# danieleschmidt/connectome-gnn-suite

Hardware: AMD Instinct MI355X
Metric: training graphs/sec, 3-layer GCN, batch=4096x360-ROI connectomes (higher is better)
Workload: dtype f32; 1 GPU; cfg4-headline-gcn-4096x360-h64; model=gcn, rois=360, ws_k=14, edges_per_graph=5040, hidden=64, layers=3, node_order=dataset, graphs_per_gpu=4096, global_batch=4096, optimizer=Adam lr1e-3 wd1e-4 (optim.Adam), impl=fused, launch=eager, bn=per-rank, rccl_ranks=0, parallelism=graph-sharded dp1

## Files before the change

### connectome_gnn_amd/csrc/fused_gcn.hip

```cpp
#include "common.h"
#include "agg_block.h"
#include "split_bf16.h"
#include "bn_tail.h"
#include "l0src.h"

#define PF_LD ld4
#define PF_ST st4
#define BW_LD ldnt4
#define BW_ST stnt4

#ifdef CGNN_STAMPS
__device__ unsigned long long g_stamps[1024 * 8 * 8];
#define CGNN_STAMP_DECL unsigned long long stamp_t_ = 0; (void)stamp_t_;
#define CGNN_STAMP_BEGIN() stamp_t_ = __builtin_amdgcn_s_memtime();
#define CGNN_STAMP(slot)                                                               \
  {                                                                                    \
    const unsigned long long now_ = __builtin_amdgcn_s_memtime();                      \
    if ((threadIdx.x & 63) == 0)                                                       \
      g_stamps[((size_t)blockIdx.x * 8 + (threadIdx.x >> 6)) * 8 + (slot)] += now_ - stamp_t_; \
    stamp_t_ = now_;                                                                   \
  }
#else
#define CGNN_STAMP_DECL
#define CGNN_STAMP_BEGIN()
// ... 340 lines not shown
  __shared__ __attribute__((aligned(16))) float bnab[2 * HID];
  __shared__ float disl[MAXR];
  const int lane = threadIdx.x & 63, wave = threadIdx.x >> 6, q = lane >> 4, j = lane & 15;
  const uint4* ent = static_cast<const uint4*>(t.ent_dst);
  constexpr int BPW = (MAXR / 16 + PF_NW - 1) / PF_NW;

  __shared__ __attribute__((aligned(16))) float b0l[FROM_P0 ? HID : 4];
  stage_split_weight<false>(wsp, W, PF_NTHR);
  for (int i = threadIdx.x; i < 2 * HID; i += PF_NTHR) bnab[i] = bn_prev[i];
  L0W w0;
  if (FROM_P0) {
    w0 = l0w_cols(l0, lane);
    for (int i = threadIdx.x; i < HID; i += PF_NTHR) b0l[i] = l0.b0[i];
  }
  const float4 bias4 = ld4(bias + 4 * j);
  double s1[4] = {0, 0, 0, 0}, s2[4] = {0, 0, 0, 0};

  constexpr int NPX = FROM_P0 ? 1 : 4;
  float4 px[BPW][NPX];
  float pd[BPW];
  auto request_block = [&](int tid, int u) {
    const int nb2 = t.tile_ptr[tid], nn2 = t.tile_ptr[tid + 1] - nb2;
    const int row = 16 * (wave + PF_NW * u) + j;
    pd[u] = 0.f;
#pragma unroll
    for (int c = 0; c < NPX; ++c) px[u][c] = make_float4(0.f, 0.f, 0.f, 0.f);
    if (row < nn2) {
      if (FROM_P0) {
        const float* src = l0.P0 + (int64_t)(nb2 + row) * L0_FP + q;
        px[u][0].x = src[0];
        px[u][0].y = src[4];
      } else {
        const float* src = Xin + (int64_t)(nb2 + row) * HID + 4 * q;
#pragma unroll
        for (int c = 0; c < NPX; ++c) px[u][c] = PF_LD(src + 16 * c);
      }
      pd[u] = t.dis[nb2 + row];
    }
  };
  auto request = [&](int tid) {
#pragma unroll
    for (int u = 0; u < BPW; ++u) request_block(tid, u);
  };
  if ((int)blockIdx.x < t.num_tiles) request(blockIdx.x);
  __syncthreads();

  for (int tid = blockIdx.x; tid < t.num_tiles; tid += gridDim.x) {
    const int base = t.tile_ptr[tid];
    const int n = t.tile_ptr[tid + 1] - base;
    const int nblk = (n + 15) >> 4;
    const int gb0 = t.tile_blk[tid];
    int boff[BPW], bwid[BPW];
#pragma unroll
    for (int k = 0; k < BPW; ++k) {
      boff[k] = bwid[k] = 0;
      const int bb = cgnn_uniform(wave) + PF_NW * k;
      if (bb < nblk) {
        boff[k] = t.blk_off_dst[gb0 + bb];
        bwid[k] = (t.blk_off_dst[gb0 + bb + 1] - boff[k]) >> 4;
      }
    }
    MetaRegs pre;
    if (wave < nblk) pre = meta_issue<true>(ent + (boff[0] >> 1), bwid[0], q, j);

    const int nxt = tid + gridDim.x;
#pragma unroll
    for (int u = 0; u < BPW; ++u) {
      const int b = wave + PF_NW * u;
      if (b >= nblk) break;
      const int row = 16 * b + j;
      const bool live = row < n;
      f32x4 acc[4] = {{0, 0, 0, 0}, {0, 0, 0, 0}, {0, 0, 0, 0}, {0, 0, 0, 0}};
#pragma unroll
      for (int ms = 0; ms < 2; ++ms) {
        float4 xc[2];
#pragma unroll
        for (int h2 = 0; h2 < 2; ++h2) {
          const int c = 2 * ms + h2;
          uint32_t keep = 0xFu;
          if (use_drop) {
            keep = drop_bits(drop, (uint32_t)(base + row), (uint32_t)(4 * c + q));
            if (mask_out && live) mask_out[(int64_t)(base + row) * 16 + 4 * c + q] = (uint8_t)keep;
          }
          float4 f;
          float4 yraw = px[u][c < NPX ? c : 0];
          if (FROM_P0) {
            const float4 bq = ld4(b0l + 16 * c + 4 * q);
            const l0_f32x4 y0 = l0_mfma(w0.a[c], w0.b[c], px[u][0].x, px[u][0].y, l0_f32x4{bq.x, bq.y, bq.z, bq.w});
            yraw = make_float4(y0[0], y0[1], y0[2], y0[3]);
          }
          xc[h2] = scale4(act4(yraw, ld4(bnab + 16 * c + 4 * q), ld4(bnab + HID + 16 * c + 4 * q),
                               keep, drop.scale, f), pd[u]);
        }
        const Split8 a = split8(xc[0], xc[1]);
#pragma unroll
        for (int tj = 0; tj < 4; ++tj) {
          const uint4 bh = wsp[((0 * 2 + ms) * 4 + tj) * 64 + lane];
          const uint4 bm = wsp[((1 * 2 + ms) * 4 + tj) * 64 + lane];
          const uint4 bl = wsp[((2 * 2 + ms) * 4 + tj) * 64 + lane];
          acc[tj] = mfma_split(a, bh, bm, bl, acc[tj]);
        }
        __builtin_amdgcn_sched_barrier(0);
      }
#pragma unroll
      for (int r = 0; r < 4; ++r)
        st4(tile + (16 * b + 4 * q + r) * HID + 4 * j, make_float4(acc[0][r], acc[1][r], acc[2][r], acc[3][r]));
      if (q == 0) disl[row] = pd[u];
      if (nxt < t.num_tiles) request_block(nxt, u);
    }
    if (nxt < t.num_tiles) {
#pragma unroll
      for (int u = 0; u < BPW; ++u)
        if (wave + PF_NW * u >= nblk) request_block(nxt, u);
    }
    __syncthreads();

#pragma unroll
    for (int u = 0; u < BPW; ++u) {
      const int b = wave + PF_NW * u;
      if (b >= nblk) break;
      float4 ag[4];
      agg_block<CGNN_PF_G, true>(tile, pre, ent + (boff[u] >> 1), bwid[u], q, j, ag);
      if (u + 1 < BPW && b + PF_NW < nblk) pre = meta_issue<true>(ent + (boff[u + 1 < BPW ? u + 1 : u] >> 1), bwid[u + 1 < BPW ? u + 1 : u], q, j);
#pragma unroll
      for (int it = 0; it < 4; ++it) {
        const int row = 16 * b + 4 * q + it;
        if (row < n) {
          const float4 a = scale4(ag[it], disl[row]);
          const float4 y = make_float4(a.x + bias4.x, a.y + bias4.y, a.z + bias4.z, a.w + bias4.w);
          PF_ST(Y + (int64_t)(base + row) * HID + 4 * j, y);
          s1[0] += y.x; s1[1] += y.y; s1[2] += y.z; s1[3] += y.w;
          s2[0] += (double)y.x * y.x; s2[1] += (double)y.y * y.y;
          s2[2] += (double)y.z * y.z; s2[3] += (double)y.w * y.w;
        }
      }
    }
    __syncthreads();
  }
  if (tail.acc) {
    double* red = reinterpret_cast<double*>(tile);
    reduce_stats<double, PF_NW>(s1, s2, red, red + PF_NW * 128);
    bn_tail_run(tail, red + PF_NW * 128, reinterpret_cast<int*>(red + PF_NW * 128 + 128), [](int) { return 0.f; });
  } else if (stat_slab) {
    reduce_stats<double, PF_NW>(s1, s2, reinterpret_cast<double*>(tile), stat_slab + (int64_t)blockIdx.x * 128);
  }
}

struct PoolIn {
  const float* dP;
  const int32_t* node_graph;
  const int32_t* gptr;
  const uint8_t* mask_cur;
};


template <int MAXR, bool FIRST, bool POOLIN, bool XP0 = false, int NW = NWAVE>
__global__ void __launch_bounds__(NW * 64) k_gcn_bwd(
    cgnn_tiles t, PoolIn pin, cgnn_l0src l0, const float* __restrict__ dZ, const float* __restrict__ Y,
    const float* __restrict__ bn, const float* __restrict__ bwc,
    const float* __restrict__ Xprev , int F0,
    const float* __restrict__ bn_prev, DropCfg drop, int use_drop,
    const uint8_t* __restrict__ mask_prev, const float* __restrict__ W,
    float* __restrict__ dZprev, double* __restrict__ s_slab, float* __restrict__ dW_slab,
    double* __restrict__ db_slab, cgnn_bn_tail tail) {
  __shared__ __attribute__((aligned(16))) float tile[MAXR * HID];
  __shared__ __attribute__((aligned(16))) float stg_all[NW * STG_FLOATS];
  __shared__ uint4 wsp[FIRST ? 1 : WSP_FRAGS];
  __shared__ float disl[MAXR];
  const int lane = threadIdx.x & 63, wave = threadIdx.x >> 6, q = lane >> 4, j = lane & 15;
  float* stg = stg_all + wave * STG_FLOATS;
  const uint4* ent = static_cast<const uint4*>(t.ent_src);

  if (!FIRST) stage_split_weight<true>(wsp, W, (NW * 64));
  __shared__ __attribute__((aligned(16))) float bnl[FIRST ? 4 : 4 * HID];
  if (!FIRST) {
    for (int i = threadIdx.x; i < 4 * HID; i += (NW * 64)) bnl[i] = bn_prev[i];
  }
  L0W w0;
  float4 b0q = make_float4(0.f, 0.f, 0.f, 0.f);
  if (XP0) {
    w0 = l0w_quad(l0, threadIdx.x & 63);
    b0q = ld4(l0.b0 + 4 * (threadIdx.x & 15));
  }
  f32x4 dw[4][FIRST ? 1 : 4];
#pragma unroll
  for (int a = 0; a < 4; ++a)
#pragma unroll
    for (int b2 = 0; b2 < (FIRST ? 1 : 4); ++b2) dw[a][b2] = f32x4{0, 0, 0, 0};
  float db[4] = {0, 0, 0, 0};
  float s1[4] = {0, 0, 0, 0}, s2[4] = {0, 0, 0, 0};
  CGNN_STAMP_DECL

  for (int tid = blockIdx.x; tid < t.num_tiles; tid += gridDim.x) {
    CGNN_STAMP_BEGIN()
    const int base = t.tile_ptr[tid];
    const int n = t.tile_ptr[tid + 1] - base;
    const int nblk = (n + 15) >> 4;
    const int gb0 = t.tile_blk[tid];
    const int uw = cgnn_uniform(wave);
    int off0 = 0, width = 0;
    if (uw < nblk) {
      off0 = t.blk_off_src[gb0 + uw];
      width = (t.blk_off_src[gb0 + uw + 1] - off0) >> 4;
    }
    MetaRegs pre;
    if (wave < nblk) pre = meta_issue<FIRST>(ent + (off0 >> 1), width, q, j);

    {
      const float4 ca = ld4(bn + 4 * j), cmean = ld4(bn + 2 * HID + 4 * j), cis = ld4(bn + 3 * HID + 4 * j);
      const float4 c1 = ld4(bwc + 4 * j), c2 = ld4(bwc + HID + 4 * j);
      const float4 cb = POOLIN ? ld4(bn + HID + 4 * j) : make_float4(0.f, 0.f, 0.f, 0.f);
#define CGNN_BWD_UNR 6
#define CGNN_BWD_UNR_POOL 6
      constexpr int UNR = POOLIN ? CGNN_BWD_UNR_POOL : CGNN_BWD_UNR;
      for (int r0 = threadIdx.x >> 4; r0 < nblk * 16; r0 += (NW * 4) * UNR) {
        float4 zb[UNR], yb[UNR];
        float dv[UNR];
        int gid[UNR];
        uint32_t kb[UNR];
#pragma unroll
        for (int u = 0; u < UNR; ++u) {
          const int row = r0 + (NW * 4) * u;
          zb[u] = yb[u] = make_float4(0.f, 0.f, 0.f, 0.f);
          dv[u] = 0.f;
          gid[u] = 0;
          kb[u] = 0xFu;
          if (row < n) {
            if (POOLIN) {
              gid[u] = pin.node_graph[base + row];
              if (use_drop) kb[u] = pin.mask_cur[(int64_t)(base + row) * 16 + j];
            } else {
              zb[u] = BW_LD(dZ + (int64_t)(base + row) * HID + 4 * j);
            }
            yb[u] = BW_LD(Y + (int64_t)(base + row) * HID + 4 * j);
            dv[u] = t.dis[base + row];
          }
        }
        if (POOLIN) {
#pragma unroll
          for (int u = 0; u < UNR; ++u) {
            const int row = r0 + (NW * 4) * u;
            if (row < n) {
              const float inv = 1.0f / ((float)(pin.gptr[gid[u] + 1] - pin.gptr[gid[u]]) + 1e-8f);
              zb[u] = scale4(ld4(pin.dP + (int64_t)gid[u] * HID + 4 * j), inv);
            }
          }
        }
#pragma unroll
        for (int u = 0; u < UNR; ++u) {
          const int row = r0 + (NW * 4) * u;
          if (row < nblk * 16) {
            float4 dy = make_float4(0.f, 0.f, 0.f, 0.f);
            if (row < n) {
              float4 dz = zb[u];
              const float4 y = yb[u];
              if (POOLIN) {
                float4 f;
                act4(y, ca, cb, kb[u], drop.scale, f);
                dz = make_float4(dz.x * f.x, dz.y * f.y, dz.z * f.z, dz.w * f.w);
              }
              dy.x = ca.x * (dz.x - c1.x - (y.x - cmean.x) * cis.x * c2.x);
              dy.y = ca.y * (dz.y - c1.y - (y.y - cmean.y) * cis.y * c2.y);
              dy.z = ca.z * (dz.z - c1.z - (y.z - cmean.z) * cis.z * c2.z);
              dy.w = ca.w * (dz.w - c1.w - (y.w - cmean.w) * cis.w * c2.w);
              db[0] += dy.x; db[1] += dy.y; db[2] += dy.z; db[3] += dy.w;
              dy = scale4(dy, dv[u]);
            }
            st4(tile + row * HID + 4 * j, dy);
            if (j == 0) disl[row] = dv[u];
          }
        }
      }
    }
    CGNN_STAMP(0)
    __syncthreads();
    CGNN_STAMP(1)

    for (int b = wave; b < nblk; b += NW) {
      float4 yp[4];
      float p0a = 0.f, p0b = 0.f;
      uint32_t keeps = 0u;
      {
        int off1 = 0, width1 = 0;
        {
          const int bn2 = cgnn_uniform(b) + NW;
          if (bn2 < nblk) {
            off1 = t.blk_off_src[gb0 + bn2];
            width1 = (t.blk_off_src[gb0 + bn2 + 1] - off1) >> 4;
          }
        }
        CGNN_STAMP(2)
        if (!FIRST) {
#pragma unroll
          for (int r = 0; r < 4; ++r) {
            const int row = 16 * b + 4 * q + r;
            yp[r] = make_float4(0.f, 0.f, 0.f, 0.f);
            if (row < n) {
                if (!XP0) yp[r] = BW_LD(Xprev + (int64_t)(base + row) * HID + 4 * j);
                uint32_t kb = 0xFu;
                if (use_drop) kb = mask_prev[(int64_t)(base + row) * 16 + j];
                keeps |= kb << (8 * r);
            }
          }
        }
        if (!FIRST && XP0 && 16 * b + j < n) {
          const float* src = l0.P0 + (int64_t)(base + 16 * b + j) * L0_FP + q;
          p0a = src[0];
          p0b = src[4];
        }
        float4 ag[4];
        agg_block<FIRST ? 4 : BWD_G, FIRST>(tile, pre, ent + (off0 >> 1), width, q, j, ag);
        CGNN_STAMP(3)
        if (XP0) {
          l0_f32x4 yt[4];
#pragma unroll
          for (int tq = 0; tq < 4; ++tq) {
            const float bt = tq == 0 ? b0q.x : tq == 1 ? b0q.y : tq == 2 ? b0q.z : b0q.w;
            yt[tq] = l0_mfma(p0a, p0b, w0.a[tq], w0.b[tq], l0_f32x4{bt, bt, bt, bt});
          }
#pragma unroll
          for (int r = 0; r < 4; ++r) yp[r] = make_float4(yt[0][r], yt[1][r], yt[2][r], yt[3][r]);
        }
#pragma unroll
        for (int it = 0; it < 4; ++it)
          st4(stg + (4 * q + it) * SLD + 4 * j, scale4(ag[it], disl[16 * b + 4 * q + it]));
        if (b + NW < nblk) pre = meta_issue<FIRST>(ent + (off1 >> 1), width1, q, j);
        off0 = off1; width = width1;
      }
      __builtin_amdgcn_wave_barrier();

      if (FIRST) {
        float xv[4];
#pragma unroll
        for (int s = 0; s < 4; ++s) {
          const int row = 16 * b + 4 * q + s;
          xv[s] = (row < n && j < F0) ? Xprev[(int64_t)(base + row) * F0 + j] : 0.f;
        }
#pragma unroll
        for (int s = 0; s < 4; ++s) {
#pragma unroll
          for (int ti = 0; ti < 4; ++ti) {
            const float av = stg[(4 * q + s) * SLD + 16 * ti + j];
            dw[ti][0] = __builtin_amdgcn_mfma_f32_16x16x4f32(av, xv[s], dw[ti][0], 0, 0, 0);
          }
        }
        __builtin_amdgcn_wave_barrier();
        CGNN_STAMP(4)
        continue;
      }

      const float4 pa = ld4(bnl + 4 * j), pb = ld4(bnl + HID + 4 * j);
#pragma unroll
      for (int s = 0; s < 4; ++s) {
        float4 f;
        const float4 x = act4(yp[s], pa, pb, (keeps >> (8 * s)) & 0xFu, drop.scale, f);
        const float bx[4] = {x.x, x.y, x.z, x.w};
#pragma unroll
        for (int ti = 0; ti < 4; ++ti) {
          const float av = stg[(4 * q + s) * SLD + 16 * ti + j];
#pragma unroll
          for (int tj = 0; tj < 4; ++tj)
            dw[ti][tj] = __builtin_amdgcn_mfma_f32_16x16x4f32(av, bx[tj], dw[ti][tj], 0, 0, 0);
        }
      }
      f32x4 dx[4] = {{0, 0, 0, 0}, {0, 0, 0, 0}, {0, 0, 0, 0}, {0, 0, 0, 0}};
#pragma unroll
      for (int ms = 0; ms < 2; ++ms) {
        const Split8 a = split8(ld4(stg + j * SLD + 16 * (2 * ms) + 4 * q),
                                ld4(stg + j * SLD + 16 * (2 * ms + 1) + 4 * q));
#pragma unroll
        for (int tj = 0; tj < 4; ++tj) {
          const uint4 bh = wsp[((0 * 2 + ms) * 4 + tj) * 64 + lane];
          const uint4 bm = wsp[((1 * 2 + ms) * 4 + tj) * 64 + lane];
          const uint4 bl = wsp[((2 * 2 + ms) * 4 + tj) * 64 + lane];
          dx[tj] = mfma_split(a, bh, bm, bl, dx[tj]);
        }
      }
      __builtin_amdgcn_wave_barrier();
      const float4 pa2 = ld4(bnl + 4 * j), pb2 = ld4(bnl + HID + 4 * j);
      const float4 pmean = ld4(bnl + 2 * HID + 4 * j), pis = ld4(bnl + 3 * HID + 4 * j);
#pragma unroll
      for (int r = 0; r < 4; ++r) {
        const int row = 16 * b + 4 * q + r;
        if (row < n) {
          float4 f;
          act4(yp[r], pa2, pb2, (keeps >> (8 * r)) & 0xFu, drop.scale, f);
          const float4 dzp = make_float4(dx[0][r] * f.x, dx[1][r] * f.y, dx[2][r] * f.z, dx[3][r] * f.w);
          BW_ST(dZprev + (int64_t)(base + row) * HID + 4 * j, dzp);
          s1[0] += dzp.x; s1[1] += dzp.y; s1[2] += dzp.z; s1[3] += dzp.w;
          s2[0] = fmaf(dzp.x, (yp[r].x - pmean.x) * pis.x, s2[0]);
          s2[1] = fmaf(dzp.y, (yp[r].y - pmean.y) * pis.y, s2[1]);
          s2[2] = fmaf(dzp.z, (yp[r].z - pmean.z) * pis.z, s2[2]);
          s2[3] = fmaf(dzp.w, (yp[r].w - pmean.w) * pis.w, s2[3]);
        }
      }
      CGNN_STAMP(4)
    }
    CGNN_STAMP(5)
    __syncthreads();
    CGNN_STAMP(6)
  }

  {
    double* red = reinterpret_cast<double*>(tile);
    __syncthreads();
    const int g = threadIdx.x >> 4;
#pragma unroll
    for (int i = 0; i < 4; ++i) red[g * 64 + 4 * j + i] = (double)db[i];
    __syncthreads();
    if (threadIdx.x < 64) {
      double s = 0.0;
      for (int g2 = 0; g2 < (NW * 64) / 16; ++g2) s += red[g2 * 64 + threadIdx.x];
      db_slab[(int64_t)blockIdx.x * 64 + threadIdx.x] = s;
    }
    __syncthreads();
  }
  if (!FIRST) {
    double* red = reinterpret_cast<double*>(tile);
    if (tail.acc) {
      reduce_stats<float, NW>(s1, s2, red, red + NW * 128);
      bn_tail_run(tail, red + NW * 128, reinterpret_cast<int*>(red + NW * 128 + 128), [](int) { return 0.f; });
    } else {
      reduce_stats<float, NW>(s1, s2, red, s_slab + (int64_t)blockIdx.x * 128);
    }
  }
  {
    constexpr int NTJ = FIRST ? 1 : 4;
    constexpr int PER = 64 * 16 * NTJ;
    float* red = tile;
    __syncthreads();
    for (int half = NW / 2; half >= 1; half >>= 1) {
      if (wave >= half && wave < 2 * half) {
        float* dst = red + (wave - half) * PER;
#pragma unroll
        for (int ti = 0; ti < 4; ++ti)
#pragma unroll
          for (int tj = 0; tj < NTJ; ++tj)
#pragma unroll
            for (int r = 0; r < 4; ++r) dst[((ti * NTJ + tj) * 4 + r) * 64 + lane] = dw[ti][tj][r];
      }
      __syncthreads();
      if (wave < half) {
        const float* src = red + wave * PER;
#pragma unroll
        for (int ti = 0; ti < 4; ++ti)
#pragma unroll
          for (int tj = 0; tj < NTJ; ++tj)
#pragma unroll
            for (int r = 0; r < 4; ++r) dw[ti][tj][r] += src[((ti * NTJ + tj) * 4 + r) * 64 + lane];
      }
      __syncthreads();
    }
    if (wave == 0) {
      constexpr int NC = FIRST ? 16 : HID;
      float* out = dW_slab + (int64_t)blockIdx.x * 64 * NC;
#pragma unroll
      for (int ti = 0; ti < 4; ++ti)
#pragma unroll
        for (int r = 0; r < 4; ++r) {
          const int o = 16 * ti + 4 * q + r;
          if (FIRST) out[o * NC + j] = dw[ti][0][r];
          else st4(out + o * NC + 4 * j, make_float4(dw[ti][0][r], dw[ti][NTJ > 1 ? 1 : 0][r],
                                                     dw[ti][NTJ > 2 ? 2 : 0][r], dw[ti][NTJ > 3 ? 3 : 0][r]));
        }
    }
  }
}

constexpr int PTHR = 256;

__global__ void __launch_bounds__(PTHR) k_pool_fwd(const float* __restrict__ Y,
                                                   const float* __restrict__ bn, DropCfg drop_in,
                                                   int use_drop, uint8_t* __restrict__ mask_out,
                                                   const int32_t* __restrict__ gptr, int B,
                                                   float* __restrict__ P, float* __restrict__ F1,
                                                   float* __restrict__ F2) {
  const DropCfg drop = drop_resolve(drop_in);
  __shared__ float red[3 * 16 * HID];
  const int j = threadIdx.x & 15, rr = threadIdx.x >> 4;
  const float4 a = ld4(bn + 4 * j), b = ld4(bn + HID + 4 * j);
  const float4 mean = ld4(bn + 2 * HID + 4 * j), is = ld4(bn + 3 * HID + 4 * j);
  for (int g = blockIdx.x; g < B; g += gridDim.x) {
    const int rbeg = gptr[g], rend = gptr[g + 1];
    float4 s = make_float4(0.f, 0.f, 0.f, 0.f), f1 = s, f2 = s;
#define CGNN_POOL_U 4
    constexpr int U = CGNN_POOL_U;
    for (int row0 = rbeg + rr; row0 < rend; row0 += 16 * U) {
      float4 yb[U];
#pragma unroll
      for (int u = 0; u < U; ++u) {
        const int row = row0 + 16 * u;
        yb[u] = row < rend ? ldnt4(Y + (int64_t)row * HID + 4 * j) : make_float4(0.f, 0.f, 0.f, 0.f);
      }
#pragma unroll
      for (int u = 0; u < U; ++u) {
        const int row = row0 + 16 * u;
        if (row < rend) {
          uint32_t keep = 0xFu;
          if (use_drop) {
            keep = drop_bits(drop, (uint32_t)row, (uint32_t)j);
            if (mask_out) mask_out[(int64_t)row * 16 + j] = (uint8_t)keep;
          }
          float4 f;
          const float4 y = yb[u];
          const float4 x = act4(y, a, b, keep, drop.scale, f);
          s.x += x.x; s.y += x.y; s.z += x.z; s.w += x.w;
          if (F1) {
            f1.x += f.x; f1.y += f.y; f1.z += f.z; f1.w += f.w;
            f2.x = fmaf(f.x, (y.x - mean.x) * is.x, f2.x); f2.y = fmaf(f.y, (y.y - mean.y) * is.y, f2.y);
            f2.z = fmaf(f.z, (y.z - mean.z) * is.z, f2.z); f2.w = fmaf(f.w, (y.w - mean.w) * is.w, f2.w);
          }
        }
      }
    }
    st4(red + rr * HID + 4 * j, s);
    if (F1) {
      st4(red + (16 + rr) * HID + 4 * j, f1);
      st4(red + (32 + rr) * HID + 4 * j, f2);
    }
    __syncthreads();
    if (threadIdx.x < HID) {
      float tot = 0.f;
#pragma unroll
      for (int k = 0; k < 16; ++k) tot += red[k * HID + threadIdx.x];
      P[(int64_t)g * HID + threadIdx.x] = tot / ((float)(rend - rbeg) + 1e-8f);
    } else if (F1 && threadIdx.x < 3 * HID) {
      const int which = threadIdx.x / HID, col = threadIdx.x % HID;
      double tot = 0.0;
#pragma unroll
      for (int k = 0; k < 16; ++k) tot += (double)red[(16 * which + k) * HID + col];
      (which == 1 ? F1 : F2)[(int64_t)g * HID + col] = (float)tot;
    }
    __syncthreads();
  }
}

__global__ void __launch_bounds__(128) k_pool_bwd_sums(const float* __restrict__ dP,
                                                       const float* __restrict__ F1,
                                                       const float* __restrict__ F2,
                                                       const int32_t* __restrict__ gptr, int B,
                                                       double* __restrict__ s_slab) {
  const int col = threadIdx.x & 63;
  const float* F = threadIdx.x < 64 ? F1 : F2;
  double acc = 0.0;
  for (int g = blockIdx.x; g < B; g += gridDim.x) {
    const float inv = 1.0f / ((float)(gptr[g + 1] - gptr[g]) + 1e-8f);
    acc += (double)(dP[(int64_t)g * HID + col] * inv) * (double)F[(int64_t)g * HID + col];
  }
  s_slab[(int64_t)blockIdx.x * 128 + threadIdx.x] = acc;
}
// ... 364 lines not shown
           tl->rng_n <= 64 && (tl->rng_n == 0 || tl->rng_state);
  return tl->dgamma && tl->dbeta && tl->bwc;
}

bool tiles_ok(const cgnn_tiles* t) {
  return t && t->num_tiles >= 0 && t->num_nodes >= 0 && t->max_tile_rows <= CGNN_FUSED_MAX_ROWS &&
         (t->num_tiles == 0 || (t->tile_ptr && t->tile_blk && t->blk_off_dst && t->ent_dst &&
                                t->blk_off_src && t->ent_src && t->dis));
}

}

extern "C" {

#ifdef CGNN_STAMPS
int cgnn_debug_stamps(unsigned long long* out_host) {
  if (hipDeviceSynchronize() != hipSuccess) return CGNN_ELAUNCH;
  if (hipMemcpyFromSymbol(out_host, HIP_SYMBOL(g_stamps), sizeof(g_stamps)) != hipSuccess) return CGNN_ELAUNCH;
  static unsigned long long zeros[1024 * 8 * 8];
  if (hipMemcpyToSymbol(HIP_SYMBOL(g_stamps), zeros, sizeof(zeros)) != hipSuccess) return CGNN_ELAUNCH;
  return CGNN_OK;
}
#endif

int cgnn_fused_grid(void) { return fused_grid(); }

int cgnn_set_fused_grid(int32_t workgroups) {
  if (workgroups < 0 || workgroups > 65535) return CGNN_EINVAL;
  g_grid_override = workgroups;
  return CGNN_OK;
}

int cgnn_gcn_fused_fwd_first(const cgnn_tiles* t, const float* X0, int32_t F0, const float* W0,
                             const float* bias, float* Y, double* stat_slab, int64_t stat_slab_bytes, void* stream) {
  if (!tiles_ok(t) || F0 <= 0 || F0 > CGNN_FUSED_MAX_F0) return t && t->max_tile_rows > CGNN_FUSED_MAX_ROWS ? CGNN_EUNSUPPORTED : CGNN_EINVAL;
  if (!X0 || !W0 || !bias || !Y) return CGNN_EINVAL;
  CGNN_NEED_BYTES(stat_slab, stat_slab_bytes, (int64_t)fused_grid() * 128 * (int64_t)sizeof(double));
  DropCfg d{};
  k_gcn_fwd<CGNN_FUSED_MAX_ROWS, true><<<fused_grid(), NTHR, 0, cgnn_stream(stream)>>>(
      *t, X0, F0, nullptr, d, 0, nullptr, W0, bias, Y, stat_slab);
  CGNN_CHECK_LAUNCH();
  return CGNN_OK;
}

int cgnn_rng_advance(uint32_t* state, int32_t n, void* stream) {
  if (!state || n <= 0 || n > 64) return CGNN_EINVAL;
  k_rng_advance<<<1, 64, 0, cgnn_stream(stream)>>>(state, n);
  CGNN_CHECK_LAUNCH();
  return CGNN_OK;
}

int cgnn_gcn_fused_fwd(const cgnn_tiles* t, const float* Yprev, const cgnn_l0src* l0,
                       const float* bn_prev, float p_drop, uint64_t seed, const uint32_t* seed_dev,
                       uint8_t* mask_out, const float* W, const float* bias, float* Y,
                       double* stat_slab, int64_t stat_slab_bytes, const cgnn_bn_tail* tail, void* stream) {
  if (!tiles_ok(t)) return t && t->max_tile_rows > CGNN_FUSED_MAX_ROWS ? CGNN_EUNSUPPORTED : CGNN_EINVAL;
  if ((!Yprev && !l0src_ok(l0)) || !bn_prev || !W || !bias || !Y || p_drop < 0.f || p_drop >= 1.f) return CGNN_EINVAL;
  if (!tail_ok(tail, 0)) return CGNN_EINVAL;
  const cgnn_bn_tail tl = tail ? *tail : cgnn_bn_tail{};
  CGNN_NEED_BYTES(stat_slab, stat_slab_bytes, (int64_t)fused_grid() * 128 * (int64_t)sizeof(double));
  int use_drop;
  DropCfg d = make_drop(p_drop, seed, &use_drop);
  d.dev_key = seed_dev;
  if (Yprev)
    k_gcn_fwd_pf<CGNN_FUSED_MAX_ROWS, false><<<fused_grid(), PF_NTHR, 0, cgnn_stream(stream)>>>(
        *t, Yprev, cgnn_l0src{}, bn_prev, d, use_drop, mask_out, W, bias, Y, stat_slab, tl);
  else
    k_gcn_fwd_pf<CGNN_FUSED_MAX_ROWS, true><<<fused_grid(), PF_NTHR, 0, cgnn_stream(stream)>>>(
        *t, nullptr, *l0, bn_prev, d, use_drop, mask_out, W, bias, Y, stat_slab, tl);
  CGNN_CHECK_LAUNCH();
  return CGNN_OK;
}

int cgnn_bn_reduce(const double* slab, int32_t rows, int32_t width, double* sums, void* stream) {
  if (!slab || !sums || rows <= 0 || width <= 0) return CGNN_EINVAL;
  k_slab_reduce<double><<<(width + 3) / 4, 256, 0, cgnn_stream(stream)>>>(slab, rows, width, sums,
                                                                        nullptr, 1, 1, 1);
  CGNN_CHECK_LAUNCH();
  return CGNN_OK;
}

int cgnn_bn_finalize(const double* sums, double count, const double* count_dev, const float* gamma,
                     const float* beta, float* running_mean, float* running_var, float momentum,
                     float eps, int32_t training, float* bn_out, const float* mean_offset, void* stream) {
  if (!gamma || !beta || !running_mean || !running_var || !bn_out) return CGNN_EINVAL;
  if (training && (!sums || (!count_dev && count <= 0.0))) return CGNN_EINVAL;
  k_bn_finalize<<<1, 64, 0, cgnn_stream(stream)>>>(sums, count, count_dev, gamma, beta, running_mean,
                                                   running_var, momentum, eps, training, bn_out, mean_offset);
  CGNN_CHECK_LAUNCH();
  return CGNN_OK;
}

int cgnn_gcn_fused_pool_fwd(const float* Y, const float* bn, float p_drop, uint64_t seed,
                            const uint32_t* seed_dev, uint8_t* mask_out, const int32_t* gptr,
                            int32_t num_graphs, float* P, float* F1, float* F2, void* stream) {
  if (num_graphs < 0 || p_drop < 0.f || p_drop >= 1.f) return CGNN_EINVAL;
  if (num_graphs == 0) return CGNN_OK;
  if (!Y || !bn || !gptr || !P || (!F1) != (!F2)) return CGNN_EINVAL;
  int use_drop;
  DropCfg d = make_drop(p_drop, seed, &use_drop);
  d.dev_key = seed_dev;
  const int grid = num_graphs < 8 * fused_grid() ? num_graphs : 8 * fused_grid();
  k_pool_fwd<<<grid, PTHR, 0, cgnn_stream(stream)>>>(Y, bn, d, use_drop, mask_out, gptr, num_graphs, P,
                                                     F1, F2);
  CGNN_CHECK_LAUNCH();
  return CGNN_OK;
}

int cgnn_gcn_fused_pool_bwd_sums(const float* dP, const float* F1, const float* F2,
                                 const int32_t* gptr, int32_t num_graphs, double* s_slab, int64_t s_slab_bytes,
                                 void* stream) {
  if (num_graphs < 0 || !dP || !F1 || !F2 || !gptr || !s_slab) return CGNN_EINVAL;
  CGNN_NEED_BYTES(s_slab, s_slab_bytes, (int64_t)fused_grid() * 128 * (int64_t)sizeof(double));
  k_pool_bwd_sums<<<fused_grid(), 128, 0, cgnn_stream(stream)>>>(dP, F1, F2, gptr, num_graphs, s_slab);
  CGNN_CHECK_LAUNCH();
  return CGNN_OK;
}

int cgnn_gcn_fused_pool_bwd(const float* dP, const float* Y, const float* bn, float p_drop,
                            const uint8_t* mask, const int32_t* gptr, int32_t num_graphs,
                            float* dZ, double* s_slab, int64_t s_slab_bytes, void* stream) {
  if (num_graphs < 0 || p_drop < 0.f || p_drop >= 1.f) return CGNN_EINVAL;
  if (!dP || !Y || !bn || !gptr || !s_slab) return CGNN_EINVAL;
  if (p_drop > 0.f && !mask) return CGNN_EINVAL;
  CGNN_NEED_BYTES(s_slab, s_slab_bytes, (int64_t)fused_grid() * 128 * (int64_t)sizeof(double));
  int use_drop;
  DropCfg d = make_drop(p_drop, 0, &use_drop);
  k_pool_bwd<<<fused_grid(), PBTHR, 0, cgnn_stream(stream)>>>(dP, Y, bn, d, use_drop, mask, gptr,
                                                             num_graphs, dZ, s_slab);
  CGNN_CHECK_LAUNCH();
  return CGNN_OK;
}

int cgnn_bn_bwd_finalize(const double* sums, double count, const double* count_dev,
                         int32_t zero_coef, float* dgamma, float* dbeta, float* bwc, void* stream) {
  if (!sums || !dgamma || !dbeta || !bwc || (!count_dev && count <= 0.0)) return CGNN_EINVAL;
  k_bn_bwd_finalize<<<1, 64, 0, cgnn_stream(stream)>>>(sums, count, count_dev, zero_coef, dgamma, dbeta, bwc);
  CGNN_CHECK_LAUNCH();
  return CGNN_OK;
}

int cgnn_gcn_fused_bwd(const cgnn_tiles* t, const float* dZ, const float* Y, const float* bn,
                       const float* bwc, const float* Yprev, const cgnn_l0src* l0,
                       const float* bn_prev, float p_drop, const uint8_t* mask_prev, const float* W,
                       float* dZprev, double* s_slab_prev, int64_t s_slab_prev_bytes, float* dW_slab, int64_t dW_slab_bytes, double* db_slab, int64_t db_slab_bytes,
                       const float* dP, const int32_t* node_graph, const int32_t* gptr,
                       const uint8_t* mask_cur, const cgnn_bn_tail* tail, void* stream) {
  if (!tiles_ok(t)) return t && t->max_tile_rows > CGNN_FUSED_MAX_ROWS ? CGNN_EUNSUPPORTED : CGNN_EINVAL;
  if (!Y || !bn || !bwc || (!Yprev && !l0src_ok(l0)) || !bn_prev || !W || !dZprev || (!s_slab_prev && !tail) ||
      !dW_slab || !db_slab || p_drop < 0.f || p_drop >= 1.f)
    return CGNN_EINVAL;
  if (!tail_ok(tail, 1)) return CGNN_EINVAL;
  const cgnn_bn_tail tl = tail ? *tail : cgnn_bn_tail{};
  if (p_drop > 0.f && !mask_prev) return CGNN_EINVAL;
  if (dP ? (!node_graph || !gptr || (p_drop > 0.f && !mask_cur)) : !dZ) return CGNN_EINVAL;
  CGNN_NEED_BYTES(s_slab_prev, s_slab_prev_bytes, (int64_t)fused_grid() * 128 * (int64_t)sizeof(double));
  CGNN_NEED_BYTES(dW_slab, dW_slab_bytes, (int64_t)fused_grid() * HID * HID * (int64_t)sizeof(float));
  CGNN_NEED_BYTES(db_slab, db_slab_bytes, (int64_t)fused_grid() * HID * (int64_t)sizeof(double));
  int use_drop;
  DropCfg d = make_drop(p_drop, 0, &use_drop);
  PoolIn pin{dP, node_graph, gptr, mask_cur};
  const cgnn_l0src src = Yprev ? cgnn_l0src{} : *l0;
#define CGNN_BWD_NW 8
#define CGNN_BWD_LAUNCH(POOL, XP)                                                                      \
  k_gcn_bwd<CGNN_FUSED_MAX_ROWS, false, POOL, XP, CGNN_BWD_NW><<<fused_grid(), CGNN_BWD_NW * 64, 0, cgnn_stream(stream)>>>( \
      *t, pin, src, dZ, Y, bn, bwc, Yprev, 0, bn_prev, d, use_drop, mask_prev, W, dZprev, s_slab_prev, \
      dW_slab, db_slab, tl)
  if (dP) { if (Yprev) CGNN_BWD_LAUNCH(true, false); else CGNN_BWD_LAUNCH(true, true); }
  else    { if (Yprev) CGNN_BWD_LAUNCH(false, false); else CGNN_BWD_LAUNCH(false, true); }
#undef CGNN_BWD_LAUNCH
  CGNN_CHECK_LAUNCH();
  return CGNN_OK;
}

int cgnn_gcn_fused_bwd_first(const cgnn_tiles* t, const float* dZ, const float* Y, const float* bn,
                             const float* bwc, const float* X0, int32_t F0, float* dW_slab, int64_t dW_slab_bytes,
                             double* db_slab, int64_t db_slab_bytes, float p_drop, const float* dP,
                             const int32_t* node_graph, const int32_t* gptr,
                             const uint8_t* mask_cur, void* stream) {
  if (!tiles_ok(t) || F0 <= 0 || F0 > CGNN_FUSED_MAX_F0) return t && t->max_tile_rows > CGNN_FUSED_MAX_ROWS ? CGNN_EUNSUPPORTED : CGNN_EINVAL;
  if (!Y || !bn || !bwc || !X0 || !dW_slab || !db_slab || p_drop < 0.f || p_drop >= 1.f) return CGNN_EINVAL;
  if (dP ? (!node_graph || !gptr || (p_drop > 0.f && !mask_cur)) : !dZ) return CGNN_EINVAL;
  CGNN_NEED_BYTES(dW_slab, dW_slab_bytes, (int64_t)fused_grid() * HID * 16 * (int64_t)sizeof(float));
  CGNN_NEED_BYTES(db_slab, db_slab_bytes, (int64_t)fused_grid() * HID * (int64_t)sizeof(double));
  int use_drop;
  DropCfg d = make_drop(dP ? p_drop : 0.f, 0, &use_drop);
  PoolIn pin{dP, node_graph, gptr, mask_cur};
  if (dP)
    k_gcn_bwd<CGNN_FUSED_MAX_ROWS, true, true><<<fused_grid(), NTHR, 0, cgnn_stream(stream)>>>(
        *t, pin, cgnn_l0src{}, dZ, Y, bn, bwc, X0, F0, nullptr, d, use_drop, nullptr, nullptr, nullptr, nullptr,
        dW_slab, db_slab, cgnn_bn_tail{});
  else
    k_gcn_bwd<CGNN_FUSED_MAX_ROWS, true, false><<<fused_grid(), NTHR, 0, cgnn_stream(stream)>>>(
        *t, pin, cgnn_l0src{}, dZ, Y, bn, bwc, X0, F0, nullptr, d, use_drop, nullptr, nullptr, nullptr, nullptr,
        dW_slab, db_slab, cgnn_bn_tail{});
  CGNN_CHECK_LAUNCH();
  return CGNN_OK;
}

int cgnn_bn_stats_finalize(const double* slab, int32_t rows, double count, const float* gamma,
                           const float* beta, float* running_mean, float* running_var,
                           float momentum, float eps, int64_t* num_batches_tracked, float* bn_out,
                           void* stream) {
  if (!slab || rows <= 0 || count <= 0.0 || !gamma || !beta || !running_mean || !running_var || !bn_out)
    return CGNN_EINVAL;
  k_bn_fwd_stats<<<HID, 256, 0, cgnn_stream(stream)>>>(
      slab, rows, count, gamma, beta, running_mean, running_var, momentum, eps,
      reinterpret_cast<long long*>(num_batches_tracked), bn_out, nullptr, 0, nullptr);
  CGNN_CHECK_LAUNCH();
  return CGNN_OK;
}

int cgnn_bn_stats_finalize_rng(const double* slab, int32_t rows, double count, const float* gamma,
                               const float* beta, float* running_mean, float* running_var,
                               float momentum, float eps, int64_t* num_batches_tracked, float* bn_out,
                               uint32_t* rng_state, int32_t rng_n, const float* mean_offset, void* stream) {
  if (!slab || rows <= 0 || count <= 0.0 || !gamma || !beta || !running_mean || !running_var || !bn_out)
    return CGNN_EINVAL;
  if (rng_n < 0 || rng_n > 64 || (rng_n > 0 && !rng_state)) return CGNN_EINVAL;
  k_bn_fwd_stats<<<HID, 256, 0, cgnn_stream(stream)>>>(
      slab, rows, count, gamma, beta, running_mean, running_var, momentum, eps,
      reinterpret_cast<long long*>(num_batches_tracked), bn_out, rng_state, rng_n, mean_offset);
  CGNN_CHECK_LAUNCH();
  return CGNN_OK;
}

int cgnn_gcn_fused_pool_bwd_finalize(const float* dP, const float* F1, const float* F2,
                                     const int32_t* gptr, int32_t num_graphs, double count,
                                     int32_t zero_coef, float* dgamma, float* dbeta, float* bwc,
                                     void* stream) {
  if (num_graphs < 0 || count <= 0.0 || !dP || !F1 || !F2 || !gptr || !dgamma || !dbeta || !bwc)
    return CGNN_EINVAL;
  k_pool_bwd_finalize<<<HID, 256, 0, cgnn_stream(stream)>>>(dP, F1, F2, gptr, num_graphs, count, zero_coef,
                                                           dgamma, dbeta, bwc);
  CGNN_CHECK_LAUNCH();
  return CGNN_OK;
}

int cgnn_bn_bwd_stats_finalize(const double* slab, int32_t rows, double count, int32_t zero_coef,
                               float* dgamma, float* dbeta, float* bwc, void* stream) {
  if (!slab || rows <= 0 || count <= 0.0 || !dgamma || !dbeta || !bwc) return CGNN_EINVAL;
  k_bn_bwd_stats<<<HID, 256, 0, cgnn_stream(stream)>>>(slab, rows, count, zero_coef, dgamma, dbeta, bwc);
  CGNN_CHECK_LAUNCH();
  return CGNN_OK;
}

int cgnn_dw_db_reduce(const float* dw_slab, const double* db_slab, int32_t rows, int32_t out_cols,
                      int32_t take_cols, float* dW, int32_t ld_dw, float* db, void* stream) {
  if (!dw_slab || !db_slab || !dW || !db || rows <= 0 || out_cols <= 0 || take_cols <= 0 ||
      take_cols > out_cols || ld_dw < take_cols)
    return CGNN_EINVAL;
  k_dw_db_reduce<<<(HID * out_cols + HID) / RD_C, RD_C * RD_G, 0, cgnn_stream(stream)>>>(dw_slab, db_slab, rows, out_cols,
                                                                 take_cols, dW, ld_dw, db);
  CGNN_CHECK_LAUNCH();
  return CGNN_OK;
}

int cgnn_dw_db_reduce_multi(const cgnn_dw_jobs* jobs, void* stream) {
  if (!jobs || jobs->n < 1 || jobs->n > CGNN_DW_MAX_JOBS) return CGNN_EINVAL;
  int total = 0;
  for (int i = 0; i < jobs->n; ++i) {
    if (!jobs->dw_slab[i] || !jobs->db_slab[i] || !jobs->dW[i] || !jobs->db[i] || jobs->rows[i] <= 0 ||
        jobs->out_cols[i] <= 0 || jobs->take_cols[i] <= 0 || jobs->take_cols[i] > jobs->out_cols[i])
      return CGNN_EINVAL;
    total += (HID * jobs->out_cols[i] + HID) / RD_C;
  }
  k_dw_db_reduce_multi<<<total, RD_C * RD_G, 0, cgnn_stream(stream)>>>(*jobs);
  CGNN_CHECK_LAUNCH();
  return CGNN_OK;
}

int cgnn_slab_reduce_f32(const float* slab, int32_t rows, int32_t out_rows, int32_t out_cols,
                         int32_t take_cols, float* out, int32_t ld_out, void* stream) {
  if (!slab || !out || rows <= 0 || out_rows <= 0 || out_cols <= 0 || take_cols <= 0 ||
      take_cols > out_cols || ld_out < take_cols)
    return CGNN_EINVAL;
  const int width = out_rows * out_cols;
  k_slab_reduce<float><<<(width + 3) / 4, 256, 0, cgnn_stream(stream)>>>(
      slab, rows, width, nullptr, out, out_cols, take_cols, ld_out);
  CGNN_CHECK_LAUNCH();
  return CGNN_OK;
}

int cgnn_slab_reduce_f32_split(const float* slab, int32_t rows, int32_t width, int32_t split, float* out,
                               float* out_tail, void* stream) {
  if (!slab || !out || !out_tail || rows <= 0 || width <= 0 || split <= 0 || split >= width) return CGNN_EINVAL;
  k_slab_reduce<float><<<(width + 3) / 4, 256, 0, cgnn_stream(stream)>>>(slab, rows, width, nullptr, out, width,
                                                                        width, width, out_tail, split);
  CGNN_CHECK_LAUNCH();
  return CGNN_OK;
}

int cgnn_slab_reduce_f64_multi(const cgnn_reduce_jobs* jobs, void* stream) {
  if (!jobs || jobs->n < 0 || jobs->n > CGNN_REDUCE_MAX_JOBS) return CGNN_EINVAL;
  if (jobs->n == 0) return CGNN_OK;
  int wmax = 0;
  for (int j = 0; j < jobs->n; ++j) {
    if (!jobs->slab[j] || !jobs->out[j] || jobs->rows[j] <= 0 || jobs->width[j] <= 0) return CGNN_EINVAL;
    wmax = jobs->width[j] > wmax ? jobs->width[j] : wmax;
  }
  k_slab_reduce_multi<<<dim3((wmax + 3) / 4, jobs->n), 256, 0, cgnn_stream(stream)>>>(*jobs);
  CGNN_CHECK_LAUNCH();
  return CGNN_OK;
}

int cgnn_slab_reduce_f64(const double* slab, int32_t rows, int32_t width, float* out, void* stream) {
  if (!slab || !out || rows <= 0 || width <= 0) return CGNN_EINVAL;
// ... 8 lines not shown
```

Baseline: 2.264 million graphs/s.

## Stage pooled readout gradients in LDS and coalesce dropout mask loads in GCN backward

```diff
diff --git a/connectome_gnn_amd/csrc/fused_gcn.hip b/connectome_gnn_amd/csrc/fused_gcn.hip
--- a/connectome_gnn_amd/csrc/fused_gcn.hip
+++ b/connectome_gnn_amd/csrc/fused_gcn.hip
@@ -516,6 +516,17 @@
   const int32_t* gptr;
   const uint8_t* mask_cur;
 };
+
+#ifndef CGNN_BWD_UNR
+#define CGNN_BWD_UNR 4
+#endif
+#ifndef CGNN_BWD_UNR_POOL
+#define CGNN_BWD_UNR_POOL 4
+#endif
+#ifndef CGNN_BWD_RO_G
+#define CGNN_BWD_RO_G 8
+#endif
+constexpr int RO_G = CGNN_BWD_RO_G;
 
 
 template <int MAXR, bool FIRST, bool POOLIN, bool XP0 = false, int NW = NWAVE>
@@ -540,6 +551,28 @@
   if (!FIRST) {
     for (int i = threadIdx.x; i < 4 * HID; i += (NW * 64)) bnl[i] = bn_prev[i];
   }
+  __shared__ __attribute__((aligned(16))) float rog[POOLIN && RO_G > 0 ? RO_G * HID : 4];
+  __shared__ int rog_g[2];
+  auto stage_readout = [&](int tt) {
+    const int nb = t.tile_ptr[tt], nn = t.tile_ptr[tt + 1] - nb;
+    const int g0 = nn > 0 ? pin.node_graph[nb] : 0;
+    const int ng = nn > 0 ? pin.node_graph[nb + nn - 1] - g0 + 1 : 0;
+    if (ng <= RO_G) {
+      for (int i = lane; i < ng * 16; i += 64) {
+        const int g = g0 + (i >> 4), c = i & 15;
+        const float inv = 1.0f / ((float)(pin.gptr[g + 1] - pin.gptr[g]) + 1e-8f);
+        st4(rog + (i >> 4) * HID + 4 * c, scale4(ld4(pin.dP + (int64_t)g * HID + 4 * c), inv));
+      }
+    }
+    if (lane == 0) {
+      rog_g[0] = g0;
+      rog_g[1] = ng <= RO_G;
+    }
+  };
+  if (POOLIN) {
+    if (cgnn_uniform(wave) == NW - 1 && (int)blockIdx.x < t.num_tiles) stage_readout(blockIdx.x);
+    __syncthreads();
+  }
   L0W w0;
   float4 b0q = make_float4(0.f, 0.f, 0.f, 0.f);
   if (XP0) {
@@ -569,13 +602,14 @@
     }
     MetaRegs pre;
     if (wave < nblk) pre = meta_issue<FIRST>(ent + (off0 >> 1), width, q, j);
+    const int nxt = tid + gridDim.x;
 
     {
       const float4 ca = ld4(bn + 4 * j), cmean = ld4(bn + 2 * HID + 4 * j), cis = ld4(bn + 3 * HID + 4 * j);
       const float4 c1 = ld4(bwc + 4 * j), c2 = ld4(bwc + HID + 4 * j);
       const float4 cb = POOLIN ? ld4(bn + HID + 4 * j) : make_float4(0.f, 0.f, 0.f, 0.f);
-#define CGNN_BWD_UNR 6
-#define CGNN_BWD_UNR_POOL 6
+      const int rg0 = POOLIN ? rog_g[0] : 0;
+      const bool rstaged = POOLIN && rog_g[1] != 0;
       constexpr int UNR = POOLIN ? CGNN_BWD_UNR_POOL : CGNN_BWD_UNR;
       for (int r0 = threadIdx.x >> 4; r0 < nblk * 16; r0 += (NW * 4) * UNR) {
         float4 zb[UNR], yb[UNR];
@@ -600,7 +634,13 @@
             dv[u] = t.dis[base + row];
           }
         }
-        if (POOLIN) {
+        if (POOLIN && rstaged) {
+#pragma unroll
+          for (int u = 0; u < UNR; ++u) {
+            const int row = r0 + (NW * 4) * u;
+            if (row < n) zb[u] = ld4(rog + (gid[u] - rg0) * HID + 4 * j);
+          }
+        } else if (POOLIN) {
 #pragma unroll
           for (int u = 0; u < UNR; ++u) {
             const int row = r0 + (NW * 4) * u;
@@ -654,17 +694,18 @@
           }
         }
         CGNN_STAMP(2)
+        uint32_t kword = 0u;
         if (!FIRST) {
+          if (16 * b + 4 * q + (j >> 2) < n) {
+            kword = 0x0F0F0F0Fu;
+            if (use_drop)
+              kword = *reinterpret_cast<const uint32_t*>(mask_prev + (int64_t)(base + 16 * b + 4 * q) * 16 + 4 * j);
+          }
 #pragma unroll
           for (int r = 0; r < 4; ++r) {
             const int row = 16 * b + 4 * q + r;
             yp[r] = make_float4(0.f, 0.f, 0.f, 0.f);
-            if (row < n) {
-                if (!XP0) yp[r] = BW_LD(Xprev + (int64_t)(base + row) * HID + 4 * j);
-                uint32_t kb = 0xFu;
-                if (use_drop) kb = mask_prev[(int64_t)(base + row) * 16 + j];
-                keeps |= kb << (8 * r);
-            }
+            if (row < n && !XP0) yp[r] = BW_LD(Xprev + (int64_t)(base + row) * HID + 4 * j);
           }
         }
         if (!FIRST && XP0 && 16 * b + j < n) {
@@ -674,6 +715,13 @@
         }
         float4 ag[4];
         agg_block<FIRST ? 4 : BWD_G, FIRST>(tile, pre, ent + (off0 >> 1), width, q, j, ag);
+        if (!FIRST) {
+#pragma unroll
+          for (int r = 0; r < 4; ++r) {
+            const uint32_t v = (uint32_t)__shfl((int)kword, 16 * q + 4 * r + (j >> 2), 64);
+            keeps |= ((v >> (8 * (j & 3))) & 0xFFu) << (8 * r);
+          }
+        }
         CGNN_STAMP(3)
         if (XP0) {
           l0_f32x4 yt[4];
@@ -760,6 +808,7 @@
       }
       CGNN_STAMP(4)
     }
+    if (POOLIN && cgnn_uniform(wave) == NW - 1 && nxt < t.num_tiles) stage_readout(nxt);
     CGNN_STAMP(5)
     __syncthreads();
     CGNN_STAMP(6)
@@ -1430,7 +1479,7 @@
     return CGNN_EINVAL;
   if (!tail_ok(tail, 1)) return CGNN_EINVAL;
   const cgnn_bn_tail tl = tail ? *tail : cgnn_bn_tail{};
-  if (p_drop > 0.f && !mask_prev) return CGNN_EINVAL;
+  if (p_drop > 0.f && (!mask_prev || (reinterpret_cast<uintptr_t>(mask_prev) & 3u))) return CGNN_EINVAL;
   if (dP ? (!node_graph || !gptr || (p_drop > 0.f && !mask_cur)) : !dZ) return CGNN_EINVAL;
   CGNN_NEED_BYTES(s_slab_prev, s_slab_prev_bytes, (int64_t)fused_grid() * 128 * (int64_t)sizeof(double));
   CGNN_NEED_BYTES(dW_slab, dW_slab_bytes, (int64_t)fused_grid() * HID * HID * (int64_t)sizeof(float));
```

After: 2.418 million graphs/s (median of 6 runs). 6.8% higher.
